# UM-ARM-Lab/pytorch_volumetric

Hardware: AMD Instinct MI355X
Metric: SDF (val+grad) queries/sec (higher is better)
Workload: dtype f32

## Files before the change

include/pvamd.h:

```cpp
#ifndef PVAMD_H
#define PVAMD_H

#include <stdint.h>

#ifdef __cplusplus
extern "C" {
#endif

#define PVAMD_ABI_VERSION 16

#define PVAMD_E_NULL      (-1)
#define PVAMD_E_SHAPE     (-2)
#define PVAMD_E_ALIGN     (-3)
#define PVAMD_E_MODE      (-4)

#define PVAMD_OOB_LOOKUP_GT_SDF 0
#define PVAMD_OOB_BOUNDING_BOX  1

#define PVAMD_RULE_VALID_ON_INDEX   1
#define PVAMD_RULE_ROUND_HALF_AWAY  2
#define PVAMD_RULE_ROUND_FLOOR_HALF 4
#define PVAMD_RULE_RES_F64          8
typedef struct pvamd_grid {
    const float* vox;
    double       dmin[3];
    double       dmax[3];
    double       dres[3];
    float        fmin[3];
    float        fmax[3];
    float        fres[3];
    float        bb_min[3];
    float        bb_max[3];
    int32_t      shape[3];
    int32_t      index_f64;
    int32_t      oob_mode;
    int32_t      finalized;
    float        vlo[3];
    float        vhi[3];
    float        inv32[3];
    float        err32[3];
    int32_t      rule;
    double       dbb_min[3];
    double       dbb_max[3];
    float        range_n2;
    float        reserved0;
} pvamd_grid_t;

#define PVAMD_TRI_REC   24
#define PVAMD_TRI_TILE  256
#define PVAMD_TRI_GROUP 16
#define PVAMD_REC_FLOATS(F) ((((F) + PVAMD_TRI_TILE - 1) / PVAMD_TRI_TILE) * PVAMD_TRI_TILE * PVAMD_TRI_REC)
#define PVAMD_TILES_FLOATS(F) ((((F) + PVAMD_TRI_TILE - 1) / PVAMD_TRI_TILE) * (4 + 4 * (PVAMD_TRI_TILE / PVAMD_TRI_GROUP)))
int64_t pvamd_mesh_rec_floats(int32_t F);
int64_t pvamd_mesh_tiles_floats(int32_t F);
typedef struct pvamd_mesh {
    const float* normal;
    const float* rec;
    const float* tiles;
    const int32_t* rec_of_face;
    int32_t      F;
    int32_t      reserved;
    double       ray_dir[3];
    uint64_t*    pair_counters;
} pvamd_mesh_t;

typedef struct pvamd_joint {
    int32_t parent;
    int32_t jtype;
    int32_t jcol;
    int32_t leaf_slot;
    float   axis[3];
    float   reserved;
    float   origin[12];
} pvamd_joint_t;

int         pvamd_abi_version(void);
const char* pvamd_build_info(void);
int         pvamd_device_count(void);

int pvamd_grid_finalize(pvamd_grid_t* grid);

int pvamd_pack_grid(const float* val, const float* grad, int64_t n, float* out, void* stream);

int pvamd_cached_query(const pvamd_grid_t* grid, const float* points, int64_t P,
                       float* out_val, float* out_grad, uint8_t* out_oob, void* stream);

#define PVAMD_CQ_KERNEL_SCALAR     0
#define PVAMD_CQ_KERNEL_DIRECT_1   1
#define PVAMD_CQ_KERNEL_DIRECT_2   2
#define PVAMD_CQ_KERNEL_DIRECT_2W  3
#define PVAMD_CQ_KERNEL_DIRECT_4   4
#define PVAMD_CQ_KERNEL_WAVE_TILE  5
#define PVAMD_CQ_KERNEL_STREAMING  6
int pvamd_cached_query_kernel(int64_t P);

int pvamd_cached_outside(const pvamd_grid_t* grid, const float* points, int64_t P, float level,
                         uint8_t* out, void* stream);

int pvamd_cached_query_f64(const pvamd_grid_t* grid, const double* points, int64_t P,
                           double* out_val, double* out_grad, uint8_t* out_oob, void* stream);
int pvamd_cached_outside_f64(const pvamd_grid_t* grid, const double* points, int64_t P, double level,
                             uint8_t* out, void* stream);
int pvamd_voxel_index_f64(const pvamd_grid_t* grid, const double* points, int64_t P,
                          int64_t* out_key, int64_t* out_flat, uint8_t* out_valid, void* stream);

int pvamd_voxel_index(const pvamd_grid_t* grid, const float* points, int64_t P,
                      int64_t* out_key, int64_t* out_flat, uint8_t* out_valid, void* stream);

int pvamd_voxel_gather_f32(const pvamd_grid_t* grid, const float* storage, const float* points, int64_t P,
                           float invalid_value, float* out, void* stream);
int pvamd_voxel_gather_u8(const pvamd_grid_t* grid, const uint8_t* storage, const float* points, int64_t P,
                          uint8_t invalid_value, uint8_t* out, void* stream);
int pvamd_voxel_scatter_f32(const pvamd_grid_t* grid, float* storage, const float* points, const float* values,
                            float scalar, int64_t P, int32_t* owner_scratch, void* stream);
int pvamd_voxel_scatter_u8(const pvamd_grid_t* grid, uint8_t* storage, const float* points, const uint8_t* values,
                           uint8_t scalar, int64_t P, int32_t* owner_scratch, void* stream);

#define PVAMD_COMPOSED_INLINE_EXACT 1
#define PVAMD_COMPOSED_FORCE_PER_LANE 2
#define PVAMD_COMPOSED_FORCE_WAVE_TILE 4
#define PVAMD_COMPOSED_NO_GROUPING 64
#define PVAMD_COMPOSED_FORCE_FUSED 128
#define PVAMD_COMPOSED_TILE_POINTS 256
#define PVAMD_COMPOSED_OUT_PACKED 32
int pvamd_composed_query(const pvamd_grid_t* grids, int32_t S, const float* tf, int32_t A,
                         const float* points, int64_t P,
                         float* out_val, float* out_grad, int32_t* out_leaf, int32_t flags, void* stream);

#define PVAMD_CO_KERNEL_PER_LANE   0
#define PVAMD_CO_KERNEL_WAVE_TILE  1
#define PVAMD_CO_KERNEL_FUSED      2
int pvamd_composed_query_kernel(int32_t A, int64_t P, int32_t flags);

int pvamd_composed_query_f64(const pvamd_grid_t* grids, int32_t S, const double* tf, int32_t A,
                             const double* points, int64_t P,
                             double* out_val, double* out_grad, int32_t* out_leaf, void* stream);

int pvamd_transform_points(const float* tf, int32_t A, const float* points, int64_t P, float* out, void* stream);
int pvamd_compose_merge(const float* tf, int32_t A, int64_t P, const float* leaf_val, const float* leaf_grad,
                        int32_t s, int32_t first, float* best_val, float* best_grad, int32_t* best_leaf, void* stream);

int pvamd_composed_query_bucketed(const pvamd_grid_t* grids, int32_t S, const float* tf, int32_t A,
                                  const float* sorted_points, const int32_t* inv, int64_t P, int64_t Pp,
                                  float* scratch, float* out_val, float* out_grad, int32_t flags, void* stream);

int64_t pvamd_group_chunk_points(void);
int64_t pvamd_group_scratch_bytes(int64_t P);
int pvamd_group_points(const float* points, int64_t P, void* scratch, void* stream);
int pvamd_composed_query_grouped(const pvamd_grid_t* grids, int32_t S, const float* tf, int32_t A, const void* scratch,
                                 int64_t P, float* out_val, float* out_grad, int32_t* out_leaf, int32_t flags, void* stream);

int pvamd_composed_query_packed(const pvamd_grid_t* grids, int32_t S, const float* tf, int32_t A, const float* points,
                                int64_t Pp, float* out_rec, int32_t flags, void* stream);
int pvamd_unpack_records(const float* rec, const int32_t* index, int64_t P, int64_t stride, int32_t A, float* out_val,
                         float* out_grad, void* stream);

int pvamd_mesh_prepare(const float* tri, const int32_t* face_id, int32_t F, float abs_margin, float* rec_out,
                       float* tiles_out, int32_t* rec_of_face_out, void* stream);

int pvamd_points_aabb(const float* points, int64_t P, float* box_out, void* stream);

int pvamd_morton_keys(const float* points, int64_t P, const float* box, int32_t* keys_out, void* stream);

#define PVAMD_MORTON_ORDER_BITS(P) ((P) >= (1 << 20) ? 21 : ((P) >= (1 << 16) ? 18 : 15))
#ifndef PVAMD_ORDER_RADIX_SORT_FROM
#define PVAMD_ORDER_RADIX_SORT_FROM (3 << 18)
#endif
int64_t pvamd_morton_order_scratch_bytes(int64_t P);
int pvamd_morton_order(const float* points, int64_t P, int32_t* order_out, int32_t* inv_out, float* sorted_points_out,
                       void* scratch, void* stream);

#define PVAMD_ORDER_KERNEL_SMALL     0
#define PVAMD_ORDER_KERNEL_COUNTING  1
#define PVAMD_ORDER_KERNEL_RADIX     2
int pvamd_morton_order_kernel(int64_t P);
int pvamd_morton_order_bits(int64_t P);

#define PVAMD_MESH_SCRATCH_GROUPS 8192
#define PVAMD_MESH_SCRATCH_SLOTS(P) ((((P) + 63) / 64) < PVAMD_MESH_SCRATCH_GROUPS ? (((P) + 63) / 64) : \
                                     ((((P) + 63) / 64) / 8 > PVAMD_MESH_SCRATCH_GROUPS ? (((P) + 63) / 64) / 8 : PVAMD_MESH_SCRATCH_GROUPS))
#define PVAMD_MESH_SMALL_POINTS 16384
#define PVAMD_MESH_SCRATCH_BYTES(P) (64 + PVAMD_MESH_SCRATCH_SLOTS(P) * (int64_t)(64 * 40 + 8 + 64) + 24 * PVAMD_MESH_SMALL_POINTS)
int64_t pvamd_mesh_scratch_bytes(int64_t P);
int64_t pvamd_mesh_small_points(void);
int pvamd_mesh_query(const pvamd_mesh_t* mesh, const float* points, const int32_t* order, int64_t P,
                     uint64_t jitter_seed, int64_t index_base, float* out_closest, float* out_dist, float* out_grad, int32_t* out_face,
                     float* out_normal, void* scratch, void* stream);

#define PVAMD_MESH_PATH_NONE        0
#define PVAMD_MESH_PATH_LISTED      1
#define PVAMD_MESH_PATH_SCAN        2
#define PVAMD_MESH_PATH_SCAN_HEAVY  3
#define PVAMD_MESH_ORDER_GIVEN      0
#define PVAMD_MESH_ORDER_INSIDE     1
#define PVAMD_MESH_ORDER_SORT_CALL  2
typedef struct pvamd_mesh_plan_t {
    int32_t path;
    int32_t order;
    int32_t groups;
    int32_t slots;
    int32_t scan_waves;
    int32_t parts;
    int32_t part_waves;
} pvamd_mesh_plan_t;
int pvamd_mesh_query_plan(int64_t P, int32_t F, int32_t has_scratch, int32_t unordered, pvamd_mesh_plan_t* plan_out);
// ... 252 lines not shown
```

pytorch_volumetric_amd/csrc/mesh.hip:

```cpp
#include "common.h"
#include "mesh_math.h"
#include "morton.h"
#include "order_small.h"
#include "wave_ops.h"

namespace pvamd {

constexpr int kRec = PVAMD_TRI_REC;
constexpr int kTile = PVAMD_TRI_TILE;
constexpr int kGroup = PVAMD_TRI_GROUP;
constexpr int kGroupsPerTile = kTile / kGroup;
static_assert(kTile == 256 && kGroup == 16 && kRec == 24, "the scan is written for 256-record tiles of six float4 planes");
enum { kPlaneSphere = 0, kPlaneU = 1, kPlaneV = 2, kPlaneA = 3, kPlaneB = 4, kPlaneC = 5 };
constexpr int kTileFloats = kTile * kRec;
PVAMD_DEV const f32x4* tile_plane(const float* rec, int tile, int plane) {
    return reinterpret_cast<const f32x4*>(rec + (int64_t)tile * kTileFloats + plane * (kTile * 4));
}
PVAMD_DEV f32x4 record_plane(const float* rec, int j, int plane) { return tile_plane(rec, j / kTile, plane)[j % kTile]; }

struct MeshArgs {
    const float* normal;
    const float* rec;
    const float* tiles;
    const int* rec_of_face;
    int F;
    double ray_dir[3];
    unsigned long long* pairs;
};
#define PVAMD_COUNT_PAIRS(m, which, n)                                                                                  \
    do {                                                                                                                \
        if ((m).pairs) {                                                                                                \
            const unsigned long long count_ = (unsigned long long)(n);  \
            if ((int)(threadIdx.x & 63) == __builtin_ctzll(__ballot(true))) atomicAdd((m).pairs + (which), count_);     \
        }                                                                                                               \
    } while (0)

struct D3 { double x, y, z; };
PVAMD_DEV D3 d3(double x, double y, double z) { return D3{x, y, z}; }
PVAMD_DEV D3 dsub(D3 a, D3 b) { return d3(a.x - b.x, a.y - b.y, a.z - b.z); }
PVAMD_DEV double ddot(D3 a, D3 b) { return a.x * b.x + a.y * b.y + a.z * b.z; }
PVAMD_DEV D3 dcross(D3 a, D3 b) { return d3(a.y * b.z - a.z * b.y, a.z * b.x - a.x * b.z, a.x * b.y - a.y * b.x); }
PVAMD_DEV D3 dscale(D3 a, double k) { return d3(a.x * k, a.y * k, a.z * k); }
PVAMD_DEV D3 dunit(D3 a, D3 fallback) {
    const double n = sqrt(ddot(a, a));
    return (n > 0.0 && n < 1e300) ? dscale(a, 1.0 / n) : fallback;
}
PVAMD_DEV double dmax3(double a, double b, double c) { return fmax(a, fmax(b, c)); }
PVAMD_DEV double dmin3(double a, double b, double c) { return fmin(a, fmin(b, c)); }

__global__ __launch_bounds__(256) void mesh_prepare_records(const float* __restrict__ tri, const int* __restrict__ face_id,
                                                            int F, float abs_margin, float* __restrict__ rec) {
    const int f = blockIdx.x * blockDim.x + threadIdx.x;
    f32x4* o = reinterpret_cast<f32x4*>(rec + (int64_t)blockIdx.x * kTileFloats) + threadIdx.x;
    if (f >= F) {
        const f32x4 zero = {0.f, 0.f, 0.f, 0.f};
        for (int pl = 0; pl < 6; ++pl) o[pl * kTile] = zero;
        return;
    }
    const float* t = tri + 9 * (int64_t)f;
    const D3 A = d3(t[0], t[1], t[2]), B = d3(t[3], t[4], t[5]), C = d3(t[6], t[7], t[8]);
    const D3 eab = dsub(B, A), ebc = dsub(C, B), eca = dsub(A, C);
    const double lab = ddot(eab, eab), lbc = ddot(ebc, ebc), lca = ddot(eca, eca);
    D3 e = eab;
    if (lbc > lab && lbc >= lca) e = ebc;
    else if (lca > lab && lca > lbc) e = eca;
    const D3 U = dunit(e, d3(1.0, 0.0, 0.0));
    const double ax = fabs(U.x), ay = fabs(U.y), az = fabs(U.z);
    const D3 axis = (ax <= ay && ax <= az) ? d3(1.0, 0.0, 0.0) : (ay <= az ? d3(0.0, 1.0, 0.0) : d3(0.0, 0.0, 1.0));
    const D3 Nd = dunit(dcross(eab, dsub(C, A)), dunit(dcross(U, axis), d3(0.0, 0.0, 1.0)));
    const D3 V = dunit(dcross(Nd, U), axis);
    const float uf[3] = {(float)U.x, (float)U.y, (float)U.z}, vf[3] = {(float)V.x, (float)V.y, (float)V.z};
    const D3 Uf = d3(uf[0], uf[1], uf[2]), Vf = d3(vf[0], vf[1], vf[2]);
    const D3 Nf = dunit(dcross(Uf, Vf), Nd);
    const D3 rb = dsub(B, A), rc = dsub(C, A);
    const double ub = ddot(Uf, rb), uc = ddot(Uf, rc), vb = ddot(Vf, rb), vc = ddot(Vf, rc), nb = ddot(Nf, rb), nc = ddot(Nf, rc);
    const double um = 0.5 * (dmin3(0.0, ub, uc) + dmax3(0.0, ub, uc)), vm = 0.5 * (dmin3(0.0, vb, vc) + dmax3(0.0, vb, vc)),
                 nm = 0.5 * (dmin3(0.0, nb, nc) + dmax3(0.0, nb, nc));
    const float cf[3] = {(float)(A.x + Uf.x * um + Vf.x * vm + Nf.x * nm), (float)(A.y + Uf.y * um + Vf.y * vm + Nf.y * nm),
                         (float)(A.z + Uf.z * um + Vf.z * vm + Nf.z * nm)};
    const D3 Cf = d3(cf[0], cf[1], cf[2]);
    const D3 qa = dsub(A, Cf), qb = dsub(B, Cf), qc = dsub(C, Cf);
    const double hu = dmax3(fabs(ddot(Uf, qa)), fabs(ddot(Uf, qb)), fabs(ddot(Uf, qc)));
    const double hv = dmax3(fabs(ddot(Vf, qa)), fabs(ddot(Vf, qb)), fabs(ddot(Vf, qc)));
    const double sl = dmax3(fabs(ddot(Nf, qa)), fabs(ddot(Nf, qb)), fabs(ddot(Nf, qc)));
    const double r = sqrt(dmax3(ddot(qa, qa), ddot(qb, qb), ddot(qc, qc)));
    o[kPlaneSphere * kTile] = f32x4{cf[0], cf[1], cf[2], (float)(r * 1.00001) + abs_margin};
    o[kPlaneU * kTile] = f32x4{uf[0], uf[1], uf[2], (float)(hu * 1.00001) + abs_margin};
    o[kPlaneV * kTile] = f32x4{vf[0], vf[1], vf[2], (float)(hv * 1.00001) + abs_margin};
    o[kPlaneA * kTile] = f32x4{t[0], t[1], t[2], __int_as_float(face_id ? face_id[f] : f)};
    o[kPlaneB * kTile] = f32x4{t[3], t[4], t[5], (float)(1.01e6 * sl * sl) + abs_margin * abs_margin};
    o[kPlaneC * kTile] = f32x4{t[6], t[7], t[8], 0.f};
}

PVAMD_DEV void enclose(bool live, float cx, float cy, float cz, float r, int width, float abs_margin, float out[4]) {
    float sx = live ? cx : 0.f, sy = live ? cy : 0.f, sz = live ? cz : 0.f, sn = live ? 1.f : 0.f;
    for (int off = width / 2; off > 0; off >>= 1) {
        sx += __shfl_xor(sx, off, 64); sy += __shfl_xor(sy, off, 64);
        sz += __shfl_xor(sz, off, 64); sn += __shfl_xor(sn, off, 64);
    }
    sn = fmaxf(sn, 1.f);
    const float mx = sx / sn, my = sy / sn, mz = sz / sn;
    float reach = 0.f;
    if (live) {
        const float dx = cx - mx, dy = cy - my, dz = cz - mz;
        reach = sqrt_rn(dx * dx + dy * dy + dz * dz) * 1.00001f + r;
    }
    for (int off = width / 2; off > 0; off >>= 1) reach = fmaxf(reach, __shfl_xor(reach, off, 64));
    out[0] = mx; out[1] = my; out[2] = mz;
    out[3] = reach * 1.00001f + abs_margin;
}

__global__ __launch_bounds__(256) void mesh_prepare_tiles(const float* __restrict__ rec, int F, float abs_margin,
                                                          float* __restrict__ tiles) {
    __shared__ float sh[4][4];
    const int tile = blockIdx.x, ntiles = gridDim.x;
    const int f = tile * kTile + threadIdx.x;
    const bool live = f < F;
    const f32x4 o = tile_plane(rec, tile, kPlaneSphere)[live ? threadIdx.x : 0];
    const float cx = o.x, cy = o.y, cz = o.z, r = o.w;
    const int wave = threadIdx.x >> 6, lane = threadIdx.x & 63;
    float g[4];
    enclose(live, cx, cy, cz, r, kGroup, abs_margin, g);
    if (live && (threadIdx.x % kGroup) == 0) {
        float* w = tiles + 4 * (int64_t)ntiles + 4 * ((int64_t)tile * kGroupsPerTile + threadIdx.x / kGroup);
        w[0] = g[0]; w[1] = g[1]; w[2] = g[2]; w[3] = g[3];
    }
    float sx = live ? cx : 0.f, sy = live ? cy : 0.f, sz = live ? cz : 0.f, sn = live ? 1.f : 0.f;
    for (int off = 32; off > 0; off >>= 1) {
        sx += __shfl_xor(sx, off, 64); sy += __shfl_xor(sy, off, 64);
        sz += __shfl_xor(sz, off, 64); sn += __shfl_xor(sn, off, 64);
    }
    if (lane == 0) { sh[wave][0] = sx; sh[wave][1] = sy; sh[wave][2] = sz; sh[wave][3] = sn; }
    __syncthreads();
    const float tn = sh[0][3] + sh[1][3] + sh[2][3] + sh[3][3];
    const float mx = (sh[0][0] + sh[1][0] + sh[2][0] + sh[3][0]) / tn;
    const float my = (sh[0][1] + sh[1][1] + sh[2][1] + sh[3][1]) / tn;
    const float mz = (sh[0][2] + sh[1][2] + sh[2][2] + sh[3][2]) / tn;
    __syncthreads();
    float reach = 0.f;
    if (live) {
        const float dx = cx - mx, dy = cy - my, dz = cz - mz;
        reach = sqrt_rn(dx * dx + dy * dy + dz * dz) * 1.00001f + r;
    }
    for (int off = 32; off > 0; off >>= 1) reach = fmaxf(reach, __shfl_xor(reach, off, 64));
    if (lane == 0) sh[wave][0] = reach;
    __syncthreads();
    if (threadIdx.x == 0) {
        float* w = tiles + 4 * (int64_t)tile;
        w[0] = mx; w[1] = my; w[2] = mz;
        w[3] = fmaxf(fmaxf(sh[0][0], sh[1][0]), fmaxf(sh[2][0], sh[3][0])) * 1.00001f + abs_margin;
    }
}

PVAMD_DEV float norm3_unfused(V3 g) {
    return sqrt_rn(add_rn(add_rn(mul_rn(g.x, g.x), mul_rn(g.y, g.y)), mul_rn(g.z, g.z)));
}

struct LaneState {
    V3 p;
    float reach;
    float reach2m, reach2x;
};

PVAMD_DEV void set_reach(LaneState& s, float reach) {
    s.reach = reach;
    s.reach2m = reach * reach * 1.00001f;
    s.reach2x = 2.00002f * reach;
}

PVAMD_DEV bool sphere_may_improve(const LaneState& s, float dist2, float r) {
    return !(dist2 > fmaf(r, fmaf(r, 1.00001f, s.reach2x), s.reach2m));
}

PVAMD_DEV bool sphere_may_hit(float dist2, float tp, float r) {
    const float perp2 = fmaf(-tp, tp, dist2);
    return !(perp2 > fmaf(r, r, 2e-6f * dist2)) && !(tp < -r);
}

PVAMD_DEV bool rect_may_improve(const LaneState& s, V3 w, float dist2, V3 fu, float hu, V3 fv, float hv, float m0) {
    const float u = dot(fu, w), v = dot(fv, w);
    const float h2 = fmaxf(fmaf(-v, v, fmaf(-u, u, dist2)), 0.f);
    const float du = fmaxf(fabsf(u) - hu, 0.f), dv = fmaxf(fabsf(v) - hv, 0.f);
    const float lb2 = fmaf(dv, dv, fmaf(du, du, h2));
    return !(lb2 > fmaf(8e-6f, dist2, s.reach2m + m0));
}

constexpr int kQueueCap = 128;
constexpr unsigned long long kBestInit = 0x7F80000000000000ull;

template <bool WITH_RAY>
struct WaveLocal {
    f32x4 sphere[64], fu[64], fv[64];
    float m0[64];
    unsigned qc[kQueueCap];
    unsigned qr[WITH_RAY ? kQueueCap : 1];
};
template <bool WITH_RAY>
struct GroupShared {
    unsigned long long best[64];
    int hits[WITH_RAY ? 64 : 1];
    int handed;
    float dir[WITH_RAY ? 192 : 1];
    float dn[WITH_RAY ? 192 : 1];
};
template <int SLICES, bool WITH_RAY>
struct MeshShared {
    GroupShared<WITH_RAY> g;
    WaveLocal<WITH_RAY> w[SLICES];
};

PVAMD_DEV float uniform(float v) { return __int_as_float(__builtin_amdgcn_readfirstlane(__float_as_int(v))); }
PVAMD_DEV V3 xyz(f32x4 v) { return v3(v.x, v.y, v.z); }

struct WaveBound {
    LaneState q;
    float rho;
    V3 dn0;
    float k, rho_k;
};

template <bool WITH_RAY>
struct Wave {
    LaneState s;
    bool live;
    V3 dn, dir;
    WaveBound wb;
    int nc, nr;
};

template <bool WITH_RAY>
PVAMD_DEV void refresh_bound(Wave<WITH_RAY>& wv) {
    const float rmax = wave_max(wv.live ? wv.s.reach : 0.f);
    set_reach(wv.wb.q, uniform((rmax + wv.wb.rho) * 1.00001f));
}

template <bool WITH_RAY>
PVAMD_DEV void pull_reach(const GroupShared<WITH_RAY>& g, Wave<WITH_RAY>& wv) {
    const float d2 = __int_as_float((int)(unsigned)(g.best[threadIdx.x & 63] >> 32));
    const float reach = fast_sqrt(d2) * 1.00001f + 1.1e-19f;
    if (reach < wv.s.reach) set_reach(wv.s, reach);
    refresh_bound(wv);
}

template <bool WITH_RAY>
PVAMD_DEV bool wave_setup(const MeshArgs& m, Wave<WITH_RAY>& wv) {
    const V3 p = wv.s.p;
    wv.live = fabsf(p.x) < INFINITY && fabsf(p.y) < INFINITY && fabsf(p.z) < INFINITY;
    wv.nc = wv.nr = 0;
    set_reach(wv.s, INFINITY);
    if (__ballot(wv.live) == 0ull) return false;
    const float lx = wave_min(wv.live ? p.x : INFINITY), hx = wave_max(wv.live ? p.x : -INFINITY);
    const float ly = wave_min(wv.live ? p.y : INFINITY), hy = wave_max(wv.live ? p.y : -INFINITY);
    const float lz = wave_min(wv.live ? p.z : INFINITY), hz = wave_max(wv.live ? p.z : -INFINITY);
    wv.wb.q.p = v3(uniform(0.5f * lx + 0.5f * hx), uniform(0.5f * ly + 0.5f * hy), uniform(0.5f * lz + 0.5f * hz));
    const V3 d = v3(p.x - wv.wb.q.p.x, p.y - wv.wb.q.p.y, p.z - wv.wb.q.p.z);
    wv.wb.rho = uniform(wave_max(wv.live ? fast_sqrt(dot(d, d)) : 0.f) * 1.00001f + 1.1e-19f);
    wv.wb.dn0 = v3(0.f, 0.f, 0.f);
    wv.wb.k = wv.wb.rho_k = 0.f;
    if (WITH_RAY) {
        const V3 a = v3((float)m.ray_dir[0], (float)m.ray_dir[1], (float)m.ray_dir[2]);
        const float inv = 1.f / sqrt_rn(dot(a, a));
        wv.wb.dn0 = v3(uniform(a.x * inv), uniform(a.y * inv), uniform(a.z * inv));
        const V3 e = v3(wv.dn.x - wv.wb.dn0.x, wv.dn.y - wv.wb.dn0.y, wv.dn.z - wv.wb.dn0.z);
        const float chord = wave_max(wv.live ? fast_sqrt(dot(e, e)) : 0.f);
        wv.wb.k = uniform(2.001f * chord + 2e-6f);
        wv.wb.rho_k = uniform(wv.wb.rho * (1.f + wv.wb.k) * 1.00001f);
    }
    set_reach(wv.wb.q, INFINITY);
    return true;
}

PVAMD_DEV bool axis_may_hit(const WaveBound& wb, V3 w, float dist2, float r) {
    const float dist = fast_sqrt(dist2) * 1.00001f + 1.1e-19f;
    return sphere_may_hit(dist2, dot(w, wb.dn0), fmaf(wb.k, dist, r + wb.rho_k));
}

PVAMD_DEV void enqueue(unsigned* q, int& n, unsigned long long mask, bool mine, int j) {
    const int lane = threadIdx.x & 63;
    if (mine) q[n + __popcll(mask & ((1ull << lane) - 1ull))] = ((unsigned)j << 6) | (unsigned)lane;
    n += __popcll(mask);
}

template <class Fn>
PVAMD_DEV void drain(unsigned* q, int& n, bool everything, Fn&& fn) {
    const int lane = threadIdx.x & 63;
    PVAMD_WAVE_SYNC();
    fn(n < 64 ? n : 64, q);
    if (n > 64) {
        const int rem = n - 64;
        if (everything) {
            fn(rem, q + 64);
            n = 0;
        } else {
            const unsigned v = lane < rem ? q[64 + lane] : 0u;
            if (lane < rem) q[lane] = v;
            n = rem;
        }
    } else {
        n = 0;
    }
    PVAMD_WAVE_SYNC();
}

template <bool WITH_RAY>
PVAMD_DEV void drain_closest(const MeshArgs& m, GroupShared<WITH_RAY>& g, WaveLocal<WITH_RAY>& wl, Wave<WITH_RAY>& wv, bool everything) {
    if (wv.nc == 0) return;
    const int lane = threadIdx.x & 63;
    drain(wl.qc, wv.nc, everything, [&](int count, const unsigned* q) {
        PVAMD_COUNT_PAIRS(m, 0, count);
        const unsigned e = lane < count ? q[lane] : 0u;
        const int owner = e & 63;
        const V3 p = v3(__shfl(wv.s.p.x, owner, 64), __shfl(wv.s.p.y, owner, 64), __shfl(wv.s.p.z, owner, 64));
        if (lane < count) {
            const int j = (int)(e >> 6);
            const f32x4 A = record_plane(m.rec, j, kPlaneA), B = record_plane(m.rec, j, kPlaneB), C = record_plane(m.rec, j, kPlaneC);
            const V3 qp = sub(closest_point_triangle(p, xyz(A), xyz(B), xyz(C)), p);
            const float d2 = dot(qp, qp);
            atomicMin(&g.best[owner], ((unsigned long long)(unsigned)__float_as_int(d2) << 32) | (unsigned)__float_as_int(A.w));
        }
    });
    pull_reach(g, wv);
}

template <bool WITH_RAY>
PVAMD_DEV void drain_rays(const MeshArgs& m, GroupShared<WITH_RAY>& g, WaveLocal<WITH_RAY>& wl, Wave<WITH_RAY>& wv, bool everything) {
    if (wv.nr == 0) return;
    const int lane = threadIdx.x & 63;
    drain(wl.qr, wv.nr, everything, [&](int count, const unsigned* q) {
        PVAMD_COUNT_PAIRS(m, 1, count);
        const unsigned e = lane < count ? q[lane] : 0u;
        const int owner = e & 63;
        const V3 p = v3(__shfl(wv.s.p.x, owner, 64), __shfl(wv.s.p.y, owner, 64), __shfl(wv.s.p.z, owner, 64));
        const V3 d = v3(__shfl(wv.dir.x, owner, 64), __shfl(wv.dir.y, owner, 64), __shfl(wv.dir.z, owner, 64));
        if (lane < count) {
            const int j = (int)(e >> 6);
            const f32x4 A = record_plane(m.rec, j, kPlaneA), B = record_plane(m.rec, j, kPlaneB), C = record_plane(m.rec, j, kPlaneC);
            if (ray_hits_triangle(p, d, xyz(A), xyz(B), xyz(C))) atomicAdd(&g.hits[owner], 1);
        }
    });
}

template <bool WITH_RAY>
PVAMD_DEV void visit_tile(const MeshArgs& m, GroupShared<WITH_RAY>& g, WaveLocal<WITH_RAY>& wl, Wave<WITH_RAY>& wv, int ti,
                          int pass_lo = 0, int pass_hi = kTile / 64) {
    const int lane = threadIdx.x & 63;
    const int ntiles = (m.F + kTile - 1) / kTile;
    const int n = min(kTile, m.F - ti * kTile);
    unsigned gm = 0u;
    {
        const bool gv = lane < kGroupsPerTile && lane * kGroup < n;
        const f32x4 gs = reinterpret_cast<const f32x4*>(m.tiles)[ntiles + ti * kGroupsPerTile + (gv ? lane : 0)];
        const V3 wc = v3(gs.x - wv.wb.q.p.x, gs.y - wv.wb.q.p.y, gs.z - wv.wb.q.p.z);
        const float dc2 = dot(wc, wc);
        bool coarse = sphere_may_improve(wv.wb.q, dc2, gs.w);
        if (WITH_RAY) coarse = coarse || axis_may_hit(wv.wb, wc, dc2, gs.w);
        unsigned todo = (unsigned)__ballot(coarse && gv);
        todo &= ((1u << (pass_hi * (64 / kGroup))) - 1u) & ~((1u << (pass_lo * (64 / kGroup))) - 1u);
        while (todo != 0u) {
            const int b = __builtin_ctz(todo);
            todo &= todo - 1u;
            const V3 ctr = v3(__int_as_float(__builtin_amdgcn_readlane(__float_as_int(gs.x), b)),
                              __int_as_float(__builtin_amdgcn_readlane(__float_as_int(gs.y), b)),
                              __int_as_float(__builtin_amdgcn_readlane(__float_as_int(gs.z), b)));
            const float r = __int_as_float(__builtin_amdgcn_readlane(__float_as_int(gs.w), b));
            const V3 w = v3(ctr.x - wv.s.p.x, ctr.y - wv.s.p.y, ctr.z - wv.s.p.z);
            const float dist2 = dot(w, w);
            bool need = sphere_may_improve(wv.s, dist2, r);
            if (WITH_RAY) need = need || sphere_may_hit(dist2, dot(w, wv.dn), r);
            if (__ballot(need && wv.live) != 0ull) gm |= 1u << b;
        }
    }
    const f32x4* P0 = tile_plane(m.rec, ti, kPlaneSphere);
    const f32x4* P1 = tile_plane(m.rec, ti, kPlaneU);
    const f32x4* P2 = tile_plane(m.rec, ti, kPlaneV);
    const f32x4* P4 = tile_plane(m.rec, ti, kPlaneB);
    for (int pass = pass_lo; pass < pass_hi; ++pass) {
        if (((gm >> (pass * (64 / kGroup))) & ((1u << (64 / kGroup)) - 1u)) == 0u) continue;
        const int idx = pass * 64 + lane;
        const f32x4 a0 = P0[idx], a1 = P1[idx], a2 = P2[idx];
        const float am0 = P4[idx].w;
        bool keep_c, keep_r = false;
        {
            const bool valid = idx < n && ((gm >> (idx / kGroup)) & 1u);
            const V3 w = v3(a0.x - wv.wb.q.p.x, a0.y - wv.wb.q.p.y, a0.z - wv.wb.q.p.z);
            const float dist2 = dot(w, w);
            keep_c = valid && sphere_may_improve(wv.wb.q, dist2, a0.w) &&
                     rect_may_improve(wv.wb.q, w, dist2, xyz(a1), a1.w, xyz(a2), a2.w, am0);
            if (WITH_RAY) keep_r = valid && axis_may_hit(wv.wb, w, dist2, a0.w);
        }
        const unsigned long long mc = __ballot(keep_c), mr = WITH_RAY ? __ballot(keep_r) : 0ull;
        unsigned long long todo = mc | mr;
        if (todo == 0ull) continue;
        PVAMD_WAVE_SYNC();
        wl.sphere[lane] = a0;
        wl.fu[lane] = a1;
        wl.fv[lane] = a2;
        wl.m0[lane] = am0;
        PVAMD_WAVE_SYNC();
        const int j0 = ti * kTile + pass * 64;
        const unsigned long long live_mask = __ballot(wv.live);
        while (todo != 0ull) {
            const int b = __builtin_ctzll(todo);
            todo &= todo - 1ull;
            const f32x4 o = wl.sphere[b];
            const V3 w = v3(o.x - wv.s.p.x, o.y - wv.s.p.y, o.z - wv.s.p.z);
            const float dist2 = dot(w, w);
            if (!WITH_RAY || ((mc >> b) & 1ull)) {
                const unsigned long long near_c = live_mask & __ballot(sphere_may_improve(wv.s, dist2, o.w));
                if (near_c != 0ull) {
                    const f32x4 u = wl.fu[b], v = wl.fv[b];
                    const unsigned long long mk = near_c & __ballot(rect_may_improve(wv.s, w, dist2, xyz(u), u.w, xyz(v), v.w, wl.m0[b]));
                    if (mk) {
                        enqueue(wl.qc, wv.nc, mk, __builtin_amdgcn_inverse_ballot_w64(mk), j0 + b);
                        if (wv.nc >= 64) drain_closest(m, g, wl, wv, false);
                    }
                }
            }
            if (WITH_RAY && ((mr >> b) & 1ull)) {
                const unsigned long long mk = live_mask & __ballot(sphere_may_hit(dist2, dot(w, wv.dn), o.w));
                if (mk) {
                    enqueue(wl.qr, wv.nr, mk, __builtin_amdgcn_inverse_ballot_w64(mk), j0 + b);
                    if (wv.nr >= 64) drain_rays(m, g, wl, wv, false);
                }
            }
        }
    }
}

template <bool WITH_RAY>
PVAMD_DEV int scan_seed(const MeshArgs& m, Wave<WITH_RAY>& wv, int part, int nparts) {
    const int lane = threadIdx.x & 63;
    const int ntiles = (m.F + kTile - 1) / kTile;
    const f32x4* tiles4 = reinterpret_cast<const f32x4*>(m.tiles);
    float bound = INFINITY, own = INFINITY;
    int nearest = -1;
    for (int base = 0; base < ntiles; base += 64) {
        const int ti = base + lane;
        if (ti < ntiles) {
            const f32x4 ts = tiles4[ti];
            const V3 w = v3(ts.x - wv.wb.q.p.x, ts.y - wv.wb.q.p.y, ts.z - wv.wb.q.p.z);
            const float b = fast_sqrt(dot(w, w)) * 1.00001f + (ts.w + 1.1e-19f);
            bound = fminf(bound, b);
            if ((nparts == 1 || (ti % nparts) == part) && (b < own || nearest < 0)) {
                own = b < own ? b : own;
                nearest = ti;
            }
        }
    }
    const float lowest = wave_min(bound);
    set_reach(wv.s, (lowest + wv.wb.rho) * 1.00001f);
    refresh_bound(wv);
    const float mine = wave_min(own);
    unsigned long long at = __ballot(nearest >= 0 && own == mine);
    if (at == 0ull) at = __ballot(nearest >= 0);
    return at ? __builtin_amdgcn_readlane(nearest, __builtin_ctzll(at)) : -1;
}

template <bool WITH_RAY>
PVAMD_DEV void greedy_reach(const MeshArgs& m, GroupShared<WITH_RAY>& g, Wave<WITH_RAY>& wv, int ti) {
    const int ntiles = (m.F + kTile - 1) / kTile;
    const f32x4* spheres = reinterpret_cast<const f32x4*>(m.tiles);
    const V3 p = wv.s.p;
    auto reach_of = [&](f32x4 sp) {
        const V3 w = v3(sp.x - p.x, sp.y - p.y, sp.z - p.z);
        return fast_sqrt(dot(w, w)) * 1.00001f + (sp.w + 1.1e-19f);
    };
    float bound = INFINITY;
    int gi = 0;
    const int ngroups = (min(kTile, m.F - ti * kTile) + kGroup - 1) / kGroup;
    for (int k = 0; k < ngroups; ++k) {
        const float b = reach_of(spheres[ntiles + ti * kGroupsPerTile + k]);
        if (b < bound) { bound = b; gi = k; }
    }
    const int j0 = ti * kTile + gi * kGroup;
    float nearest = INFINITY;
    int jn = -1;
    for (int k = 0; k < kGroup; ++k) {
        if (j0 + k < m.F) {
            const float b = reach_of(record_plane(m.rec, j0 + k, kPlaneSphere));
            if (b < nearest) { nearest = b; jn = j0 + k; }
        }
    }
    PVAMD_COUNT_PAIRS(m, 0, __popcll(__ballot(jn >= 0 && wv.live)));
    if (jn >= 0 && wv.live) {
        const f32x4 A = record_plane(m.rec, jn, kPlaneA), B = record_plane(m.rec, jn, kPlaneB), C = record_plane(m.rec, jn, kPlaneC);
        const V3 qp = sub(closest_point_triangle(p, xyz(A), xyz(B), xyz(C)), p);
        const float d2 = dot(qp, qp);
        atomicMin(&g.best[threadIdx.x & 63], ((unsigned long long)(unsigned)__float_as_int(d2) << 32) | (unsigned)__float_as_int(A.w));
    }
    bound = fminf(bound, nearest) * 1.00001f;
    if (bound < wv.s.reach) set_reach(wv.s, bound);
    pull_reach(g, wv);
}

template <bool WITH_RAY>
PVAMD_DEV void scan_tiles(const MeshArgs& m, GroupShared<WITH_RAY>& g, WaveLocal<WITH_RAY>& wl, Wave<WITH_RAY>& wv, int skip,
                          int part, int nparts, int pass_lo = 0, int pass_hi = kTile / 64) {
    const int lane = threadIdx.x & 63;
    const int ntiles = (m.F + kTile - 1) / kTile;
    const f32x4* tiles4 = reinterpret_cast<const f32x4*>(m.tiles);
    for (int base = 0; base < ntiles; base += 64) {
        const int ti = base + lane;
        const bool mine = ti < ntiles && ti != skip && (nparts == 1 || (ti % nparts) == part);
        const f32x4 ts = tiles4[mine ? ti : 0];
        const V3 w = v3(ts.x - wv.wb.q.p.x, ts.y - wv.wb.q.p.y, ts.z - wv.wb.q.p.z);
        const float dist2 = dot(w, w);
        const bool ray = WITH_RAY && mine && axis_may_hit(wv.wb, w, dist2, ts.w);
        const float lower = mine ? fast_sqrt(dist2) - ts.w : INFINITY;
        unsigned long long done = 0ull;
        for (;;) {
            pull_reach(g, wv);
            const bool need = mine && (ray || sphere_may_improve(wv.wb.q, dist2, ts.w));
            const unsigned long long todo = __ballot(need) & ~done;
            if (todo == 0ull) break;
            const float key = ((todo >> lane) & 1ull) ? lower : INFINITY;
            const unsigned long long at = __ballot(key == wave_min(key)) & todo;
            const int t = __builtin_ctzll(at ? at : todo);
            done |= 1ull << t;
            const V3 ctr = v3(__int_as_float(__builtin_amdgcn_readlane(__float_as_int(ts.x), t)),
                              __int_as_float(__builtin_amdgcn_readlane(__float_as_int(ts.y), t)),
                              __int_as_float(__builtin_amdgcn_readlane(__float_as_int(ts.z), t)));
            const float r = __int_as_float(__builtin_amdgcn_readlane(__float_as_int(ts.w), t));
            const V3 wl_ = v3(ctr.x - wv.s.p.x, ctr.y - wv.s.p.y, ctr.z - wv.s.p.z);
            const float d2 = dot(wl_, wl_);
            bool mine_too = sphere_may_improve(wv.s, d2, r);
            if (WITH_RAY) mine_too = mine_too || sphere_may_hit(d2, dot(wl_, wv.dn), r);
            if (__ballot(mine_too && wv.live) == 0ull) continue;
            visit_tile<WITH_RAY>(m, g, wl, wv, base + t, pass_lo, pass_hi);
        }
    }
}

template <bool WITH_RAY>
PVAMD_DEV void scan_finish(const MeshArgs& m, GroupShared<WITH_RAY>& g, WaveLocal<WITH_RAY>& wl, Wave<WITH_RAY>& wv) {
    drain_closest(m, g, wl, wv, true);
    if (WITH_RAY) drain_rays(m, g, wl, wv, true);
}

template <bool WITH_RAY>
PVAMD_DEV bool scan_begin(const MeshArgs& m, GroupShared<WITH_RAY>& g, Wave<WITH_RAY>& wv, int wave, uint64_t seed,
                          int64_t jitter_index, const unsigned long long* start, const float* __restrict__ drawn = nullptr,
                          const float* __restrict__ bound = nullptr) {
    const int lane = threadIdx.x & 63;
    if (wave == 0) {
        g.best[lane] = start ? *start : kBestInit;
        if (WITH_RAY) {
            g.hits[lane] = 0;
            const V3 dir = drawn ? v3(drawn[3 * lane], drawn[3 * lane + 1], drawn[3 * lane + 2])
                                 : jitter_dir(m.ray_dir, seed, jitter_index);
            const float inv_len = 1.f / sqrt_rn(dot(dir, dir));
            g.dir[3 * lane] = dir.x; g.dir[3 * lane + 1] = dir.y; g.dir[3 * lane + 2] = dir.z;
            g.dn[3 * lane] = dir.x * inv_len; g.dn[3 * lane + 1] = dir.y * inv_len; g.dn[3 * lane + 2] = dir.z * inv_len;
        }
    }
    __syncthreads();
    wv.dir = wv.dn = v3(0.f, 0.f, 0.f);
    if (WITH_RAY) {
        wv.dir = v3(g.dir[3 * lane], g.dir[3 * lane + 1], g.dir[3 * lane + 2]);
        wv.dn = v3(g.dn[3 * lane], g.dn[3 * lane + 1], g.dn[3 * lane + 2]);
    }
    return bound ? load_bound(bound, wv) : wave_setup(m, wv);
}

struct HandOver {
    int* count;
    int* entries;
    unsigned long long* best;
    int* hits;
    float* dir;
    float* reach;
    float* pts;
    unsigned long long* p_best;
    float* p_dir;
    float* p_reach;
    float* bound;
    int cap;
};
constexpr int kBoundFloats = 16;
constexpr int kSmallPoints = PVAMD_MESH_SMALL_POINTS;
static_assert(PVAMD_MESH_SMALL_POINTS <= kOrderSmallPoints, "an unordered query is sorted by ONE workgroup (order_small_block), which drops the points beyond its capacity");
constexpr int kHandOverHeader = 64;
struct HandOverLayout {
    size_t entries, best, hits, dir, reach, bound, pts;
    size_t p_best, p_dir, p_reach;
    size_t bytes;
};
constexpr HandOverLayout hand_over_layout(int64_t cap) {
    const size_t slots = (size_t)cap, lanes = slots * 64, small = (size_t)kSmallPoints;
    HandOverLayout l = {};
    l.entries = kHandOverHeader;
    l.best = l.entries + slots * 2 * sizeof(int);
    l.hits = l.best + lanes * sizeof(unsigned long long);
    l.dir = l.hits + lanes * sizeof(int);
    l.reach = l.dir + lanes * 3 * sizeof(float);
    l.bound = l.reach + lanes * sizeof(float);
    l.pts = l.bound + slots * kBoundFloats * sizeof(float);
    l.p_best = l.pts + lanes * 3 * sizeof(float);
    l.p_dir = l.p_best + small * sizeof(unsigned long long);
    l.p_reach = l.p_dir + small * 3 * sizeof(float);
    l.bytes = l.p_reach + small * sizeof(float);
    return l;
}
static_assert(hand_over_layout(PVAMD_MESH_SCRATCH_SLOTS(0)).bytes == PVAMD_MESH_SCRATCH_BYTES(0) &&
              hand_over_layout(PVAMD_MESH_SCRATCH_SLOTS(1)).bytes == PVAMD_MESH_SCRATCH_BYTES(1),
              "PVAMD_MESH_SCRATCH_BYTES is not the hand-over layout's total");
static_assert(hand_over_layout(0).bytes - hand_over_layout(0).p_best == (size_t)kSmallPoints * (sizeof(unsigned long long) + 4 * sizeof(float)),
              "the by-point part holds one (best, dir, reach) per point of the largest unordered query");

static HandOver hand_over(void* scratch, int cap) {
    const HandOverLayout l = hand_over_layout(cap);
    char* base = reinterpret_cast<char*>(scratch);
    HandOver h;
    h.count = reinterpret_cast<int*>(base);
    h.entries = reinterpret_cast<int*>(base + l.entries);
    h.best = reinterpret_cast<unsigned long long*>(base + l.best);
    h.hits = reinterpret_cast<int*>(base + l.hits);
    h.dir = reinterpret_cast<float*>(base + l.dir);
    h.reach = reinterpret_cast<float*>(base + l.reach);
    h.bound = reinterpret_cast<float*>(base + l.bound);
    h.pts = reinterpret_cast<float*>(base + l.pts);
    h.p_best = reinterpret_cast<unsigned long long*>(base + l.p_best);
    h.p_dir = reinterpret_cast<float*>(base + l.p_dir);
    h.p_reach = reinterpret_cast<float*>(base + l.p_reach);
    h.cap = scratch ? cap : 0;
    return h;
}
constexpr int kHeavy32nds = 6;
constexpr int kHeavyMinTiles = 128;
constexpr int kHeavyParts = 32;

PVAMD_DEV void store_bound(float* __restrict__ b, const WaveBound& wb, bool any_live) {
    if ((threadIdx.x & 63) != 0) return;
    b[0] = wb.q.p.x; b[1] = wb.q.p.y; b[2] = wb.q.p.z; b[3] = wb.rho;
    b[4] = wb.dn0.x; b[5] = wb.dn0.y; b[6] = wb.dn0.z; b[7] = wb.k;
    b[8] = wb.rho_k; b[9] = any_live ? 1.f : 0.f;
    b[10] = wb.q.reach;
}
template <bool WITH_RAY>
PVAMD_DEV bool part_has_work(const MeshArgs& m, const float* __restrict__ b, int part, int nparts) {
    if (uniform(b[9]) == 0.f) return false;
    WaveBound wb;
    wb.q.p = v3(uniform(b[0]), uniform(b[1]), uniform(b[2]));
    wb.rho = uniform(b[3]);
    wb.dn0 = v3(uniform(b[4]), uniform(b[5]), uniform(b[6]));
    wb.k = uniform(b[7]);
    wb.rho_k = uniform(b[8]);
    set_reach(wb.q, uniform(b[10]));
    const int lane = threadIdx.x & 63;
    const int ntiles = (m.F + kTile - 1) / kTile;
    const f32x4* tiles4 = reinterpret_cast<const f32x4*>(m.tiles);
    for (int base = part; base < ntiles; base += 64 * nparts) {
        const int ti = base + lane * nparts;
        const f32x4 ts = tiles4[ti < ntiles ? ti : 0];
        const V3 w = v3(ts.x - wb.q.p.x, ts.y - wb.q.p.y, ts.z - wb.q.p.z);
        const float dist2 = dot(w, w);
        bool need = sphere_may_improve(wb.q, dist2, ts.w);
        if (WITH_RAY) need = need || axis_may_hit(wb, w, dist2, ts.w);
        if (__ballot(need && ti < ntiles) != 0ull) return true;
    }
    return false;
}
template <bool WITH_RAY>
PVAMD_DEV bool load_bound(const float* __restrict__ b, Wave<WITH_RAY>& wv) {
    const V3 p = wv.s.p;
    wv.live = fabsf(p.x) < INFINITY && fabsf(p.y) < INFINITY && fabsf(p.z) < INFINITY;
    wv.nc = wv.nr = 0;
    set_reach(wv.s, INFINITY);
    wv.wb.q.p = v3(uniform(b[0]), uniform(b[1]), uniform(b[2]));
    wv.wb.rho = uniform(b[3]);
    wv.wb.dn0 = v3(uniform(b[4]), uniform(b[5]), uniform(b[6]));
    wv.wb.k = uniform(b[7]);
    wv.wb.rho_k = uniform(b[8]);
    set_reach(wv.wb.q, INFINITY);
    return uniform(b[9]) != 0.f;
}

template <bool WITH_RAY>
PVAMD_DEV int flagged_tiles(const MeshArgs& m, const Wave<WITH_RAY>& wv) {
    const int lane = threadIdx.x & 63;
    const int ntiles = (m.F + kTile - 1) / kTile;
// ... 775 lines not shown
```

pytorch_volumetric_amd/csrc/mesh_math.h:

```cpp
#pragma once
#include <hip/hip_runtime.h>
#include <stdint.h>
#include "exact_math.h"

namespace pvamd {

#ifndef PVAMD_DEV
#define PVAMD_DEV __device__ __forceinline__
#endif

struct V3 {
    float x, y, z;
};

PVAMD_DEV V3 v3(float x, float y, float z) { return V3{x, y, z}; }
PVAMD_DEV V3 sub(V3 a, V3 b) { return V3{sub_rn(a.x, b.x), sub_rn(a.y, b.y), sub_rn(a.z, b.z)}; }
PVAMD_DEV float dot(V3 a, V3 b) { return fmaf(a.z, b.z, fmaf(a.y, b.y, mul_rn(a.x, b.x))); }
PVAMD_DEV V3 cross(V3 a, V3 b) {
    return V3{fmaf(a.y, b.z, -mul_rn(a.z, b.y)), fmaf(a.z, b.x, -mul_rn(a.x, b.z)),
              fmaf(a.x, b.y, -mul_rn(a.y, b.x))};
}
PVAMD_DEV V3 madd(float s, V3 d, V3 o) { return V3{fmaf(s, d.x, o.x), fmaf(s, d.y, o.y), fmaf(s, d.z, o.z)}; }

PVAMD_DEV V3 closest_point_triangle(V3 p, V3 a, V3 b, V3 c) {
    const V3 ab = sub(b, a), ac = sub(c, a), ap = sub(p, a);
    const float d1 = dot(ab, ap), d2 = dot(ac, ap);
    if (d1 <= 0.f && d2 <= 0.f) return a;
    const V3 bp = sub(p, b);
    const float d3 = dot(ab, bp), d4 = dot(ac, bp);
    if (d3 >= 0.f && d4 <= d3) return b;
    const V3 cp = sub(p, c);
    const float d5 = dot(ab, cp), d6 = dot(ac, cp);
    if (d6 >= 0.f && d5 <= d6) return c;
    const float vc = fmaf(d1, d4, -mul_rn(d3, d2));
    if (vc <= 0.f && d1 >= 0.f && d3 <= 0.f) {
        return madd(div_rn(d1, sub_rn(d1, d3)), ab, a);
    }
    const float vb = fmaf(d5, d2, -mul_rn(d1, d6));
    if (vb <= 0.f && d2 >= 0.f && d6 <= 0.f) {
        return madd(div_rn(d2, sub_rn(d2, d6)), ac, a);
    }
    const float va = fmaf(d3, d6, -mul_rn(d5, d4));
    const float d43 = sub_rn(d4, d3), d56 = sub_rn(d5, d6);
    if (va <= 0.f && d43 >= 0.f && d56 >= 0.f) {
        return madd(div_rn(d43, add_rn(d43, d56)), sub(c, b), b);
    }
    const float denom = div_rn(1.f, add_rn(add_rn(va, vb), vc));
    const float v = mul_rn(vb, denom), w = mul_rn(vc, denom);
    return madd(w, ac, madd(v, ab, a));
}

PVAMD_DEV int ray_hits_triangle(V3 org, V3 dir, V3 v0, V3 v1, V3 v2) {
    const V3 e1 = sub(v0, v1), e2 = sub(v2, v0);
    const V3 Ng = cross(e2, e1);
    const V3 C = sub(v0, org);
    const V3 R = cross(C, dir);
    const float den = dot(Ng, dir);
    const float absden = fabsf(den);
    const float sgn = den < 0.f ? -1.f : 1.f;
    const float U = mul_rn(dot(R, e2), sgn);
    const float V = mul_rn(dot(R, e1), sgn);
    const float T = mul_rn(dot(Ng, C), sgn);
    const bool hit = (den != 0.f) && (U >= 0.f) && (V >= 0.f) && (add_rn(U, V) <= absden) && (T > 0.f);
    return hit ? 1 : 0;
}

PVAMD_DEV uint64_t splitmix64(uint64_t z) {
    z += 0x9E3779B97F4A7C15ull;
    z = (z ^ (z >> 30)) * 0xBF58476D1CE4E5B9ull;
    z = (z ^ (z >> 27)) * 0x94D049BB133111EBull;
    return z ^ (z >> 31);
}

PVAMD_DEV float jitter_normal(uint64_t seed, int64_t index, int c) {
    int s = 0;
#pragma unroll
    for (int k = 0; k < 3; ++k) {
        const uint64_t h = splitmix64(seed ^ splitmix64((uint64_t)index * 9u + (uint64_t)(c * 3 + k)));
        s += (int)(h & 0xFFFF) + (int)((h >> 16) & 0xFFFF) + (int)((h >> 32) & 0xFFFF) + (int)((h >> 48) & 0xFFFF);
    }
    return mul_rn((float)(s - 393210), 1.0f / 65536.0f);
}

PVAMD_DEV V3 jitter_dir(const double ray_dir[3], uint64_t seed, int64_t index) {
    return V3{(float)__fma_rn(1e-4, (double)jitter_normal(seed, index, 0), ray_dir[0]),
              (float)__fma_rn(1e-4, (double)jitter_normal(seed, index, 1), ray_dir[1]),
              (float)__fma_rn(1e-4, (double)jitter_normal(seed, index, 2), ray_dir[2])};
}

}
```

Baseline: 214.3 billion.

## Add oriented bounding boxes per tile and group to tighten mesh culling

Precomputes an oriented bounding box, built in double precision from the summed face normal, for every 16-triangle group and every 256-triangle tile, stored after the existing spheres. The tile and group traversal now adds a box lower-bound test after the sphere test, and tracks the ray-hit mask separately from the distance mask so rays and distance queries prune independently. This is meant to cut the number of candidate triangles visited, at the cost of more tile metadata, extra constant loads and ballots per group, and a serial per-thread box build in the prepare kernel.

```diff
diff --git a/include/pvamd.h b/include/pvamd.h
--- a/include/pvamd.h
+++ b/include/pvamd.h
@@ -50,7 +50,9 @@
 #define PVAMD_TRI_TILE  256
 #define PVAMD_TRI_GROUP 16
 #define PVAMD_REC_FLOATS(F) ((((F) + PVAMD_TRI_TILE - 1) / PVAMD_TRI_TILE) * PVAMD_TRI_TILE * PVAMD_TRI_REC)
-#define PVAMD_TILES_FLOATS(F) ((((F) + PVAMD_TRI_TILE - 1) / PVAMD_TRI_TILE) * (4 + 4 * (PVAMD_TRI_TILE / PVAMD_TRI_GROUP)))
+#define PVAMD_TRI_BOX   16
+#define PVAMD_TILES_FLOATS(F) ((((F) + PVAMD_TRI_TILE - 1) / PVAMD_TRI_TILE) * \
+                               ((4 + PVAMD_TRI_BOX) * (1 + PVAMD_TRI_TILE / PVAMD_TRI_GROUP)))
 int64_t pvamd_mesh_rec_floats(int32_t F);
 int64_t pvamd_mesh_tiles_floats(int32_t F);
 typedef struct pvamd_mesh {
diff --git a/pytorch_volumetric_amd/csrc/mesh.hip b/pytorch_volumetric_amd/csrc/mesh.hip
--- a/pytorch_volumetric_amd/csrc/mesh.hip
+++ b/pytorch_volumetric_amd/csrc/mesh.hip
@@ -13,6 +13,13 @@
 static_assert(kTile == 256 && kGroup == 16 && kRec == 24, "the scan is written for 256-record tiles of six float4 planes");
 enum { kPlaneSphere = 0, kPlaneU = 1, kPlaneV = 2, kPlaneA = 3, kPlaneB = 4, kPlaneC = 5 };
 constexpr int kTileFloats = kTile * kRec;
+constexpr int kBoxFloats = PVAMD_TRI_BOX;
+static_assert(kBoxFloats == 16, "a box is four float4s");
+static_assert(PVAMD_TILES_FLOATS(kTile) == 4 + 4 * kGroupsPerTile + kBoxFloats * (1 + kGroupsPerTile), "spheres, then boxes, per tile");
+PVAMD_DEV int64_t tile_box_at(int ntiles, int ti) { return (int64_t)ntiles * (1 + kGroupsPerTile) + (int64_t)ti * (kBoxFloats / 4); }
+PVAMD_DEV int64_t group_box_at(int ntiles, int ti, int b) {
+    return (int64_t)ntiles * (1 + kGroupsPerTile + kBoxFloats / 4) + ((int64_t)ti * kGroupsPerTile + b) * (kBoxFloats / 4);
+}
 PVAMD_DEV const f32x4* tile_plane(const float* rec, int tile, int plane) {
     return reinterpret_cast<const f32x4*>(rec + (int64_t)tile * kTileFloats + plane * (kTile * 4));
 }
@@ -110,6 +117,69 @@
     out[3] = reach * 1.00001f + abs_margin;
 }
 
+PVAMD_DEV float round_up(double d) {
+    const float f = (float)d;
+    return (double)f < d ? nextafterf(f, INFINITY) : f;
+}
+
+PVAMD_DEV void enclose_box(const float* __restrict__ rec, int tile, int lo, int hi, float abs_margin, f32x4* __restrict__ out) {
+    const f32x4* PA = tile_plane(rec, tile, kPlaneA);
+    const f32x4* PB = tile_plane(rec, tile, kPlaneB);
+    const f32x4* PC = tile_plane(rec, tile, kPlaneC);
+    if (hi <= lo) {
+        const f32x4 zero = {0.f, 0.f, 0.f, 0.f};
+        for (int k = 0; k < kBoxFloats / 4; ++k) out[k] = zero;
+        return;
+    }
+    D3 sum = d3(0.0, 0.0, 0.0);
+    double area = 0.0;
+    for (int k = lo; k < hi; ++k) {
+        const D3 A = d3(PA[k].x, PA[k].y, PA[k].z), B = d3(PB[k].x, PB[k].y, PB[k].z), C = d3(PC[k].x, PC[k].y, PC[k].z);
+        const D3 c = dcross(dsub(B, A), dsub(C, A));
+        sum = d3(sum.x + c.x, sum.y + c.y, sum.z + c.z);
+        area += sqrt(ddot(c, c));
+    }
+    const double len = sqrt(ddot(sum, sum));
+    const D3 N = (len > 1e-6 * area && len < 1e300) ? dscale(sum, 1.0 / len) : d3(0.0, 0.0, 1.0);
+    const double ax = fabs(N.x), ay = fabs(N.y), az = fabs(N.z);
+    const D3 axis = (ax <= ay && ax <= az) ? d3(1.0, 0.0, 0.0) : (ay <= az ? d3(0.0, 1.0, 0.0) : d3(0.0, 0.0, 1.0));
+    const D3 U = dunit(dsub(axis, dscale(N, ddot(axis, N))), d3(1.0, 0.0, 0.0));
+    const D3 V = dcross(N, U);
+    const float uf[3] = {(float)U.x, (float)U.y, (float)U.z}, vf[3] = {(float)V.x, (float)V.y, (float)V.z},
+                nf[3] = {(float)N.x, (float)N.y, (float)N.z};
+    const D3 Uf = d3(uf[0], uf[1], uf[2]), Vf = d3(vf[0], vf[1], vf[2]), Nf = d3(nf[0], nf[1], nf[2]);
+    const D3 O = d3(PA[lo].x, PA[lo].y, PA[lo].z);
+    double ulo = 0.0, uhi = 0.0, vlo = 0.0, vhi = 0.0, nlo = 0.0, nhi = 0.0;
+    for (int k = lo; k < hi; ++k) {
+        const f32x4 q[3] = {PA[k], PB[k], PC[k]};
+        for (int c = 0; c < 3; ++c) {
+            const D3 x = dsub(d3(q[c].x, q[c].y, q[c].z), O);
+            const double pu = ddot(Uf, x), pv = ddot(Vf, x), pn = ddot(Nf, x);
+            ulo = fmin(ulo, pu); uhi = fmax(uhi, pu);
+            vlo = fmin(vlo, pv); vhi = fmax(vhi, pv);
+            nlo = fmin(nlo, pn); nhi = fmax(nhi, pn);
+        }
+    }
+    const double um = 0.5 * (ulo + uhi), vm = 0.5 * (vlo + vhi), nm = 0.5 * (nlo + nhi);
+    const float cf[3] = {(float)(O.x + Uf.x * um + Vf.x * vm + Nf.x * nm), (float)(O.y + Uf.y * um + Vf.y * vm + Nf.y * nm),
+                         (float)(O.z + Uf.z * um + Vf.z * vm + Nf.z * nm)};
+    const D3 Cf = d3(cf[0], cf[1], cf[2]);
+    double hu = 0.0, hv = 0.0, hn = 0.0;
+    for (int k = lo; k < hi; ++k) {
+        const f32x4 q[3] = {PA[k], PB[k], PC[k]};
+        for (int c = 0; c < 3; ++c) {
+            const D3 x = dsub(d3(q[c].x, q[c].y, q[c].z), Cf);
+            hu = fmax(hu, fabs(ddot(Uf, x)));
+            hv = fmax(hv, fabs(ddot(Vf, x)));
+            hn = fmax(hn, fabs(ddot(Nf, x)));
+        }
+    }
+    out[0] = f32x4{cf[0], cf[1], cf[2], round_up(hu * 1.00001) + abs_margin};
+    out[1] = f32x4{uf[0], uf[1], uf[2], round_up(hv * 1.00001) + abs_margin};
+    out[2] = f32x4{vf[0], vf[1], vf[2], round_up(hn * 1.00001) + abs_margin};
+    out[3] = f32x4{nf[0], nf[1], nf[2], 0.f};
+}
+
 __global__ __launch_bounds__(256) void mesh_prepare_tiles(const float* __restrict__ rec, int F, float abs_margin,
                                                           float* __restrict__ tiles) {
     __shared__ float sh[4][4];
@@ -150,23 +220,20 @@
         w[0] = mx; w[1] = my; w[2] = mz;
         w[3] = fmaxf(fmaxf(sh[0][0], sh[1][0]), fmaxf(sh[2][0], sh[3][0])) * 1.00001f + abs_margin;
     }
+    const int n = max(0, min(kTile, F - tile * kTile));
+    f32x4* boxes = reinterpret_cast<f32x4*>(tiles);
+    if (threadIdx.x < kGroupsPerTile) {
+        const int b = threadIdx.x;
+        enclose_box(rec, tile, min(b * kGroup, n), min((b + 1) * kGroup, n), abs_margin, boxes + group_box_at(ntiles, tile, b));
+    } else if (threadIdx.x == kGroupsPerTile) {
+        enclose_box(rec, tile, 0, n, abs_margin, boxes + tile_box_at(ntiles, tile));
+    }
 }
 
 PVAMD_DEV float norm3_unfused(V3 g) {
     return sqrt_rn(add_rn(add_rn(mul_rn(g.x, g.x), mul_rn(g.y, g.y)), mul_rn(g.z, g.z)));
 }
 
-struct LaneState {
-    V3 p;
-    float reach;
-    float reach2m, reach2x;
-};
-
-PVAMD_DEV void set_reach(LaneState& s, float reach) {
-    s.reach = reach;
-    s.reach2m = reach * reach * 1.00001f;
-    s.reach2x = 2.00002f * reach;
-}
 
 PVAMD_DEV bool sphere_may_improve(const LaneState& s, float dist2, float r) {
     return !(dist2 > fmaf(r, fmaf(r, 1.00001f, s.reach2x), s.reach2m));
@@ -340,13 +407,22 @@
     });
 }
 
+typedef const __attribute__((address_space(4))) f32x4 ConstantF4;
+PVAMD_DEV bool box_near(const MeshArgs& m, int64_t at, const LaneState& s) {
+    const ConstantF4* box = (const ConstantF4*)(reinterpret_cast<const f32x4*>(m.tiles) + at);
+    const f32x4 c = box[0], u = box[1], v = box[2], n = box[3];
+    const V3 w = v3(c.x - s.p.x, c.y - s.p.y, c.z - s.p.z);
+    return box_may_improve(s, w, dot(w, w), xyz(u), c.w, xyz(v), u.w, xyz(n), v.w);
+}
+
 template <bool WITH_RAY>
 PVAMD_DEV void visit_tile(const MeshArgs& m, GroupShared<WITH_RAY>& g, WaveLocal<WITH_RAY>& wl, Wave<WITH_RAY>& wv, int ti,
                           int pass_lo = 0, int pass_hi = kTile / 64) {
     const int lane = threadIdx.x & 63;
     const int ntiles = (m.F + kTile - 1) / kTile;
     const int n = min(kTile, m.F - ti * kTile);
-    unsigned gm = 0u;
+    unsigned gm = 0u, gr = 0u;
+    const unsigned long long live_mask = __ballot(wv.live);
     {
         const bool gv = lane < kGroupsPerTile && lane * kGroup < n;
         const f32x4 gs = reinterpret_cast<const f32x4*>(m.tiles)[ntiles + ti * kGroupsPerTile + (gv ? lane : 0)];
@@ -365,9 +441,9 @@
             const float r = __int_as_float(__builtin_amdgcn_readlane(__float_as_int(gs.w), b));
             const V3 w = v3(ctr.x - wv.s.p.x, ctr.y - wv.s.p.y, ctr.z - wv.s.p.z);
             const float dist2 = dot(w, w);
-            bool need = sphere_may_improve(wv.s, dist2, r);
-            if (WITH_RAY) need = need || sphere_may_hit(dist2, dot(w, wv.dn), r);
-            if (__ballot(need && wv.live) != 0ull) gm |= 1u << b;
+            if (WITH_RAY && (live_mask & __ballot(sphere_may_hit(dist2, dot(w, wv.dn), r))) != 0ull) gr |= 1u << b;
+            if ((live_mask & __ballot(sphere_may_improve(wv.s, dist2, r))) == 0ull) continue;
+            if ((live_mask & __ballot(box_near(m, group_box_at(ntiles, ti, b), wv.s))) != 0ull) gm |= 1u << b;
         }
     }
     const f32x4* P0 = tile_plane(m.rec, ti, kPlaneSphere);
@@ -375,18 +451,17 @@
     const f32x4* P2 = tile_plane(m.rec, ti, kPlaneV);
     const f32x4* P4 = tile_plane(m.rec, ti, kPlaneB);
     for (int pass = pass_lo; pass < pass_hi; ++pass) {
-        if (((gm >> (pass * (64 / kGroup))) & ((1u << (64 / kGroup)) - 1u)) == 0u) continue;
+        if ((((gm | gr) >> (pass * (64 / kGroup))) & ((1u << (64 / kGroup)) - 1u)) == 0u) continue;
         const int idx = pass * 64 + lane;
         const f32x4 a0 = P0[idx], a1 = P1[idx], a2 = P2[idx];
         const float am0 = P4[idx].w;
         bool keep_c, keep_r = false;
         {
-            const bool valid = idx < n && ((gm >> (idx / kGroup)) & 1u);
             const V3 w = v3(a0.x - wv.wb.q.p.x, a0.y - wv.wb.q.p.y, a0.z - wv.wb.q.p.z);
             const float dist2 = dot(w, w);
-            keep_c = valid && sphere_may_improve(wv.wb.q, dist2, a0.w) &&
+            keep_c = idx < n && ((gm >> (idx / kGroup)) & 1u) && sphere_may_improve(wv.wb.q, dist2, a0.w) &&
                      rect_may_improve(wv.wb.q, w, dist2, xyz(a1), a1.w, xyz(a2), a2.w, am0);
-            if (WITH_RAY) keep_r = valid && axis_may_hit(wv.wb, w, dist2, a0.w);
+            if (WITH_RAY) keep_r = idx < n && ((gr >> (idx / kGroup)) & 1u) && axis_may_hit(wv.wb, w, dist2, a0.w);
         }
         const unsigned long long mc = __ballot(keep_c), mr = WITH_RAY ? __ballot(keep_r) : 0ull;
         unsigned long long todo = mc | mr;
@@ -398,7 +473,6 @@
         wl.m0[lane] = am0;
         PVAMD_WAVE_SYNC();
         const int j0 = ti * kTile + pass * 64;
-        const unsigned long long live_mask = __ballot(wv.live);
         while (todo != 0ull) {
             const int b = __builtin_ctzll(todo);
             todo &= todo - 1ull;
@@ -523,9 +597,11 @@
             const float r = __int_as_float(__builtin_amdgcn_readlane(__float_as_int(ts.w), t));
             const V3 wl_ = v3(ctr.x - wv.s.p.x, ctr.y - wv.s.p.y, ctr.z - wv.s.p.z);
             const float d2 = dot(wl_, wl_);
-            bool mine_too = sphere_may_improve(wv.s, d2, r);
-            if (WITH_RAY) mine_too = mine_too || sphere_may_hit(d2, dot(wl_, wv.dn), r);
-            if (__ballot(mine_too && wv.live) == 0ull) continue;
+            const unsigned long long live_mask = __ballot(wv.live);
+            bool mine_too = (live_mask & __ballot(sphere_may_improve(wv.s, d2, r))) != 0ull &&
+                            (live_mask & __ballot(box_near(m, tile_box_at(ntiles, base + t), wv.s))) != 0ull;
+            if (WITH_RAY) mine_too = mine_too || (live_mask & __ballot(sphere_may_hit(d2, dot(wl_, wv.dn), r))) != 0ull;
+            if (!mine_too) continue;
             visit_tile<WITH_RAY>(m, g, wl, wv, base + t, pass_lo, pass_hi);
         }
     }
diff --git a/pytorch_volumetric_amd/csrc/mesh_math.h b/pytorch_volumetric_amd/csrc/mesh_math.h
--- a/pytorch_volumetric_amd/csrc/mesh_math.h
+++ b/pytorch_volumetric_amd/csrc/mesh_math.h
@@ -65,6 +65,26 @@
     return hit ? 1 : 0;
 }
 
+struct LaneState {
+    V3 p;
+    float reach;
+    float reach2m, reach2x;
+};
+
+PVAMD_DEV void set_reach(LaneState& s, float reach) {
+    s.reach = reach;
+    s.reach2m = reach * reach * 1.00001f;
+    s.reach2x = 2.00002f * reach;
+}
+
+PVAMD_DEV bool box_may_improve(const LaneState& s, V3 w, float dist2, V3 fu, float hu, V3 fv, float hv, V3 fn, float hn) {
+    const float a = fmaxf(fabsf(dot(fu, w)) - hu, 0.f);
+    const float b = fmaxf(fabsf(dot(fv, w)) - hv, 0.f);
+    const float c = fmaxf(fabsf(dot(fn, w)) - hn, 0.f);
+    const float lb2 = fmaf(c, c, fmaf(b, b, mul_rn(a, a)));
+    return !(lb2 > fmaf(1e-6f, dist2, s.reach2m));
+}
+
 PVAMD_DEV uint64_t splitmix64(uint64_t z) {
     z += 0x9E3779B97F4A7C15ull;
     z = (z ^ (z >> 30)) * 0xBF58476D1CE4E5B9ull;
```

Result: no change. 215.2 billion, median of 4 (+0.4%).
